# emmanuel-marty/zultra

Hardware: AMD Instinct MI355X
Metric: input MB/s, gzip 64 KiB max-blocks, enwik8-sized text, bit-exact vs CPU zultra (higher is better)
Workload: dtype u8/int32

## Files before the change

include/zultra_hip.h:

```cpp
#ifndef ZULTRA_HIP_H
#define ZULTRA_HIP_H

#include <stddef.h>
#include <stdint.h>

#ifdef __cplusplus
extern "C" {
#endif

typedef struct zultra_hip_ctx_s zultra_hip_ctx_t;

typedef struct zultra_hip_block_s {
   uint64_t win_off;
   uint32_t prev;
   uint32_t n;
} zultra_hip_block_t;

typedef struct zultra_hip_subblock_s {
   uint32_t block;
   uint32_t start;
   uint32_t size;
   uint32_t is_dynamic;
   int32_t static_cost;
   int32_t dynamic_cost;
// ... 19 lines not shown

double zultra_hip_copy_bandwidth(size_t nbytes, int iters);

zultra_hip_ctx_t *zultra_hip_create(int device, uint32_t max_block_size, uint32_t max_blocks);
void zultra_hip_destroy(zultra_hip_ctx_t *ctx);
const char *zultra_hip_last_error(const zultra_hip_ctx_t *ctx);

void zultra_hip_ctx_info(const zultra_hip_ctx_t *ctx, int *device, uint32_t *max_block_size, uint32_t *max_blocks, size_t *device_bytes);
size_t zultra_hip_context_bytes_on(int device, uint32_t max_block_size, uint32_t max_blocks);
size_t zultra_hip_context_bytes(uint32_t max_block_size, uint32_t max_blocks);

void *zultra_hip_staging(zultra_hip_ctx_t *ctx, int which, size_t size);

size_t zultra_hip_data_capacity(const zultra_hip_ctx_t *ctx);

int zultra_hip_compress_blocks(zultra_hip_ctx_t *ctx, const void *data, size_t data_size, int data_on_device,
                               const zultra_hip_block_t *blocks, uint32_t nblocks);

const zultra_hip_subblock_t *zultra_hip_subblocks(const zultra_hip_ctx_t *ctx, uint32_t *count);
const uint8_t *zultra_hip_payload(const zultra_hip_ctx_t *ctx, size_t *size);
void zultra_hip_last_timing(const zultra_hip_ctx_t *ctx, zultra_hip_timing_t *t);

typedef struct zultra_hip_stats_s {
   uint64_t positions, huge_positions;
   uint32_t blocks, subblocks, tasks, huge_tasks;
   uint32_t cut_tasks, cut_segments;
   uint32_t cut_redone;
   uint32_t runs;
   uint32_t settled_passes;
   uint32_t settled_kib;
   uint32_t cut_demoted;
   uint32_t runs_without_chain_kernels;
   uint32_t batches_rerun;
} zultra_hip_stats_t;
void zultra_hip_last_stats(const zultra_hip_ctx_t *ctx, zultra_hip_stats_t *out);

uint32_t zultra_hip_mf_chunk(const zultra_hip_ctx_t *ctx, uint32_t window_size, uint32_t *max_notes);

int zultra_hip_chain_trace(zultra_hip_ctx_t *ctx, uint64_t *out, uint32_t *slots);

int zultra_hip_cut_tasks(zultra_hip_ctx_t *ctx, uint32_t run, uint32_t *out, uint32_t cap);

int zultra_hip_get_matches(zultra_hip_ctx_t *ctx, uint32_t block, uint16_t *out);
int zultra_hip_get_splits(zultra_hip_ctx_t *ctx, uint32_t block, int *out );
int zultra_hip_get_parse(zultra_hip_ctx_t *ctx, uint32_t block, uint16_t *out);

typedef struct zultra_hip_bitstate_s {
   uint32_t acc;
   uint32_t nacc;
} zultra_hip_bitstate_t;

size_t zultra_hip_stitch(zultra_hip_bitstate_t *state, const zultra_hip_subblock_t *subs, uint32_t nsubs,
                         const uint8_t *payload, const uint8_t *raw, const uint64_t *raw_off, uint32_t max_block_size,
                         int final_block, uint8_t *out, size_t out_cap);
size_t zultra_hip_stitch_finish(zultra_hip_bitstate_t *state, uint8_t *out, size_t out_cap);

int zultra_hip_stitch_device(zultra_hip_ctx_t *ctx, zultra_hip_bitstate_t *state, int final_block, uint64_t *end_bit);
int zultra_hip_stitch_with_batch(zultra_hip_ctx_t *ctx, int enable, uint32_t phase, int final_block);
int zultra_hip_stitch_phase_table(zultra_hip_ctx_t *ctx, uint64_t *end_bits , uint32_t *failed_mask);
const void *zultra_hip_stream_device(const zultra_hip_ctx_t *ctx);
int zultra_hip_stream_read(zultra_hip_ctx_t *ctx, void *out, size_t offset, size_t nbytes);
int zultra_hip_stream_write(zultra_hip_ctx_t *ctx, const void *in, size_t offset, size_t nbytes);

#define ZULTRA_HIP_VERIFY_OK 0
typedef struct zultra_hip_verify_s {
   uint32_t bad_subblocks;
   uint32_t first_bad;
   uint32_t reason;
// ... 77 lines not shown
```

zultra_amd/_ffi.py:

```python
import ctypes as C

import numpy as np

ZULTRA_OK = 0
ZULTRA_STREAM_END = 1
ZULTRA_ERROR_SRC = -1
ZULTRA_ERROR_DST = -2
ZULTRA_ERROR_DICTIONARY = -3
ZULTRA_ERROR_MEMORY = -4
ZULTRA_ERROR_COMPRESSION = -5

FLAG_DEFLATE = 0
FLAG_ZLIB = 1
FLAG_GZIP = 2

CONTINUE = 0
FINALIZE = 1

_u8p = C.POINTER(C.c_uint8)
_SIZE_MAX = C.c_size_t(-1).value


class ZultraError(RuntimeError):
    pass


class _Stream(C.Structure):
    _fields_ = [("next_in", C.c_void_p), ("avail_in", C.c_size_t), ("total_in", C.c_ulonglong),
                ("next_out", C.c_void_p), ("avail_out", C.c_size_t), ("total_out", C.c_ulonglong),
                ("zalloc", C.c_void_p), ("zfree", C.c_void_p), ("opaque", C.c_void_p),
                ("state", C.c_void_p), ("adler", C.c_uint)]


class Block(C.Structure):
    _fields_ = [("win_off", C.c_uint64), ("prev", C.c_uint32), ("n", C.c_uint32)]


class SubBlock(C.Structure):
    _fields_ = [("block", C.c_uint32), ("start", C.c_uint32), ("size", C.c_uint32), ("is_dynamic", C.c_uint32),
                ("static_cost", C.c_int32), ("dynamic_cost", C.c_int32), ("failed", C.c_uint32), ("reserved", C.c_uint32),
                ("nbits", C.c_uint64), ("bits_off", C.c_uint64)]


class Timing(C.Structure):
    _fields_ = [(k, C.c_float) for k in ("h2d_ms", "matchfinder_ms", "tokenize_split_ms", "encode_ms", "d2h_ms", "total_ms",
                                         "group_ms", "frontier_ms", "stitch_ms", "init_ms", "parse_ms", "build_ms", "post_ms", "emit_ms", "head_ms", "tail_ms")]


class Stats(C.Structure):
    _fields_ = [("positions", C.c_uint64), ("huge_positions", C.c_uint64), ("blocks", C.c_uint32), ("subblocks", C.c_uint32),
                ("tasks", C.c_uint32), ("huge_tasks", C.c_uint32), ("cut_tasks", C.c_uint32), ("cut_segments", C.c_uint32),
                ("cut_redone", C.c_uint32), ("runs", C.c_uint32), ("settled_passes", C.c_uint32), ("settled_kib", C.c_uint32), ("cut_demoted", C.c_uint32),
                ("runs_without_chain_kernels", C.c_uint32), ("batches_rerun", C.c_uint32)]


class BitState(C.Structure):
    _fields_ = [("acc", C.c_uint32), ("nacc", C.c_uint32)]


class Verify(C.Structure):
    _fields_ = [("bad_subblocks", C.c_uint32), ("first_bad", C.c_uint32), ("reason", C.c_uint32), ("block", C.c_uint32),
                ("input_off", C.c_uint64), ("stream_bit", C.c_uint64), ("verified_bytes", C.c_uint64)]


class InflateItem(C.Structure):
    _fields_ = [("src_off", C.c_uint64), ("src_size", C.c_uint64), ("dst_off", C.c_uint64), ("dst_cap", C.c_uint64)]


class InflateResult(C.Structure):
    _fields_ = [("reason", C.c_uint32), ("blocks", C.c_uint32), ("out_size", C.c_uint64), ("src_used", C.c_uint64)]


class MemberResult(C.Structure):
    _fields_ = [("reason", C.c_uint32), ("blocks", C.c_uint32), ("out_size", C.c_uint64), ("src_used", C.c_uint64), ("head_size", C.c_uint32), ("check", C.c_uint32)]


class IndexResult(C.Structure):
    _fields_ = [("members", C.c_uint32), ("stop", C.c_uint32), ("out_size", C.c_uint64), ("src_used", C.c_uint64), ("tiles", C.c_uint32), ("tiles_rewalked", C.c_uint32)]


MEMBER_DTYPE = [("off", "<u8"), ("size", "<u8"), ("check", "<u4"), ("flags", "<u4")]
FRAME_BGZF = 4
ZIP_ENTRY_DTYPE = [("local_off", "<u8"), ("comp_size", "<u4"), ("size", "<u4"), ("crc32", "<u4"), ("name_len", "<u4")]
ZIP_EMPTY = 0xFFFFFFFF
MEMBER_RESULT_DTYPE = [("reason", "<u4"), ("blocks", "<u4"), ("out_size", "<u8"), ("src_used", "<u8"), ("head_size", "<u4"), ("check", "<u4")]


EXPORTS = [
    "zultra_stream_init", "zultra_stream_set_dictionary", "zultra_stream_compress", "zultra_stream_end",
    "zultra_memory_bound", "zultra_memory_compress", "zultra_memory_compress_dict", "zultra_set_device", "zultra_set_devices",
    "zultra_frame_get_header_size", "zultra_frame_encode_header", "zultra_frame_init_checksum",
    "zultra_frame_update_checksum", "zultra_frame_get_footer_size", "zultra_frame_encode_footer",
    "zultra_dictionary_load", "zultra_dictionary_free",
    "zultra_hip_device_count", "zultra_hip_selftest", "zultra_hip_traffic_probe", "zultra_hip_create", "zultra_hip_destroy", "zultra_hip_last_error",
    "zultra_hip_data_capacity", "zultra_hip_compress_blocks", "zultra_hip_subblocks", "zultra_hip_payload",
    "zultra_hip_last_timing", "zultra_hip_get_matches", "zultra_hip_get_splits", "zultra_hip_get_parse",
    "zultra_hip_stitch", "zultra_hip_stitch_finish",
    "zultra_hip_stitch_device", "zultra_hip_stitch_phase_table", "zultra_hip_stream_device", "zultra_hip_stream_read", "zultra_hip_block_crc32", "zultra_crc32_append", "zultra_crc32_append_many",
    "zultra_hip_create_files", "zultra_hip_compress_files", "zultra_hip_stitch_files", "zultra_hip_staging",
    "zultra_hip_block_adler32", "zultra_adler32_append", "zultra_hip_copy_bandwidth", "zultra_hip_last_stats", "zultra_hip_mf_chunk",
    "zultra_hip_ctx_info", "zultra_hip_context_bytes", "zultra_hip_context_bytes_on", "zultra_release_cached_contexts", "zultra_hip_chain_trace", "zultra_hip_cut_tasks", "zultra_hip_stitch_with_batch",
    "zultra_set_verify", "zultra_verified_bytes", "zultra_hip_verify_device", "zultra_hip_last_verify_ms", "zultra_hip_stream_write",
    "zultra_memory_decompress", "zultra_hip_inflate_streams", "zultra_memory_decompress_dict", "zultra_hip_inflate_streams_dict",
    "zultra_memory_decompress_batch", "zultra_hip_inflate_members",
    "zultra_hip_index_members", "zultra_hip_inflate_file", "zultra_memory_decompress_members",
    "zultra_hip_frame_members", "zultra_hip_last_frame_ms", "zultra_memory_bound_bgzf", "zultra_memory_compress_bgzf", "zultra_memory_compress_batch",
    "zultra_hip_zip_members", "zultra_hip_zip_device", "zultra_hip_zip_read", "zultra_hip_last_zip_ms",
    "zultra_zip_end_records", "zultra_memory_bound_zip", "zultra_memory_compress_zip",
]


def _as_u8(data):
    if isinstance(data, np.ndarray):
        return np.ascontiguousarray(data, dtype=np.uint8)
    return np.frombuffer(bytes(data), dtype=np.uint8)


class Lib:
    def __init__(self, path, allow_missing=()):
        self.path = path
        L = self.L = C.CDLL(path)
        missing = [n for n in EXPORTS if not hasattr(L, n) and n not in allow_missing]
        if missing:
            raise ZultraError("%s does not export %s" % (path, missing))
        L.zultra_stream_init.argtypes = [C.POINTER(_Stream), C.c_uint, C.c_uint]
        L.zultra_stream_init.restype = C.c_int
        L.zultra_stream_set_dictionary.argtypes = [C.POINTER(_Stream), C.c_void_p, C.c_int]
        L.zultra_stream_set_dictionary.restype = C.c_int
        L.zultra_stream_compress.argtypes = [C.POINTER(_Stream), C.c_int]
        L.zultra_stream_compress.restype = C.c_int
        L.zultra_stream_end.argtypes = [C.POINTER(_Stream)]
        L.zultra_stream_end.restype = None
        L.zultra_memory_bound.argtypes = [C.c_size_t, C.c_uint, C.c_uint]
# ... 12 lines not shown
        L.zultra_frame_get_header_size.argtypes = [C.c_uint, C.c_void_p, C.c_int]
        L.zultra_frame_get_footer_size.argtypes = [C.c_uint]
        L.zultra_hip_device_count.restype = C.c_int
        L.zultra_hip_create.argtypes = [C.c_int, C.c_uint32, C.c_uint32]
        L.zultra_hip_create.restype = C.c_void_p
        L.zultra_hip_destroy.argtypes = [C.c_void_p]
        L.zultra_hip_last_error.argtypes = [C.c_void_p]
        L.zultra_hip_last_error.restype = C.c_char_p
        L.zultra_hip_data_capacity.argtypes = [C.c_void_p]
        L.zultra_hip_data_capacity.restype = C.c_size_t
        L.zultra_hip_compress_blocks.argtypes = [C.c_void_p, C.c_void_p, C.c_size_t, C.c_int, C.POINTER(Block), C.c_uint32]
        L.zultra_hip_compress_blocks.restype = C.c_int
        L.zultra_hip_subblocks.argtypes = [C.c_void_p, C.POINTER(C.c_uint32)]
        L.zultra_hip_subblocks.restype = C.POINTER(SubBlock)
        L.zultra_hip_payload.argtypes = [C.c_void_p, C.POINTER(C.c_size_t)]
        L.zultra_hip_payload.restype = _u8p
        L.zultra_hip_last_timing.argtypes = [C.c_void_p, C.POINTER(Timing)]
        L.zultra_hip_get_matches.argtypes = [C.c_void_p, C.c_uint32, C.c_void_p]
        L.zultra_hip_get_splits.argtypes = [C.c_void_p, C.c_uint32, C.POINTER(C.c_int)]
        L.zultra_hip_get_parse.argtypes = [C.c_void_p, C.c_uint32, C.c_void_p]
        L.zultra_hip_stitch.argtypes = [C.POINTER(BitState), C.POINTER(SubBlock), C.c_uint32, C.c_void_p, C.c_void_p,
                                        C.POINTER(C.c_uint64), C.c_uint32, C.c_int, C.c_void_p, C.c_size_t]
        L.zultra_hip_stitch.restype = C.c_size_t
        L.zultra_hip_stitch_finish.argtypes = [C.POINTER(BitState), C.c_void_p, C.c_size_t]
        L.zultra_hip_stitch_finish.restype = C.c_size_t

    def device_count(self):
        return self.L.zultra_hip_device_count()

    def traffic_probe(self, nbytes):
        self.L.zultra_hip_traffic_probe.argtypes = [C.c_size_t]
        return self.L.zultra_hip_traffic_probe(nbytes)

    def copy_bandwidth(self, nbytes=1 << 30, iters=5):
        self.L.zultra_hip_copy_bandwidth.argtypes = [C.c_size_t, C.c_int]
        self.L.zultra_hip_copy_bandwidth.restype = C.c_double
        return self.L.zultra_hip_copy_bandwidth(nbytes, iters)

    def memory_bound(self, n, flags, max_block=0):
        return self.L.zultra_memory_bound(n, flags, max_block)

    def memory_compress(self, data, flags, max_block=0, dictionary=None, cap=None):
        data = _as_u8(data)
        if cap is None:
            cap = self.memory_bound(len(data), flags, max_block) + 16
        out = np.empty(max(cap, 1), dtype=np.uint8)
        if dictionary is not None and len(dictionary):
            d = _as_u8(dictionary)
            r = self.L.zultra_memory_compress_dict(data.ctypes.data, len(data), out.ctypes.data, cap, flags, max_block, d.ctypes.data, len(d))
        else:
            r = self.L.zultra_memory_compress(data.ctypes.data, len(data), out.ctypes.data, cap, flags, max_block)
        if r == _SIZE_MAX:
            return None
        return out[:r].tobytes()

    def memory_compress_into(self, data, flags, max_block, out):
        data = _as_u8(data)
        r = self.L.zultra_memory_compress(data.ctypes.data, len(data), out.ctypes.data, len(out), flags, max_block)
        return None if r == _SIZE_MAX else int(r)

    def memory_decompress(self, data, flags, max_out):
        data = _as_u8(data)
        out = np.empty(max(max_out, 1), dtype=np.uint8)
        f = self.L.zultra_memory_decompress
        f.argtypes = [C.c_void_p, C.c_size_t, C.c_void_p, C.c_size_t, C.c_uint]
        f.restype = C.c_size_t
# ... 549 lines not shown
```

zultra_amd/csrc/zh_device.hip:

```cpp
#include <zh_platform.h>

#include <stdio.h>
#include <stdlib.h>
#include <string.h>

#include <algorithm>
#include <mutex>
#include <vector>

#include "../../include/zultra_hip.h"
#include "zh_common.h"
#include "zh_host.h"
#include "zh_encode.h"
#include "zh_huffman.h"
#include "zh_matchfinder.h"
#include "zh_parse.h"
#include "zh_parse_chain.h"
#include "zh_parse_lanes.h"
#include "zh_split.h"
#include "zh_stitch.h"
#include "zh_frame.h"
#include "zh_zip.h"
#include "zh_verify.h"

// ... 97 lines not shown
   zh_bets_t bets;
   uint32_t streams_respread;
   uint32_t grid_cap;
   uint32_t mf_lds_cap;
   uint32_t *d_pay;
   uint32_t *d_tok_pos;
   uint16_t *d_tok_info;
   uint32_t *d_ntok, *d_split_tok, *d_split_cnt, *d_sub_base;
   uint32_t *d_chunkmax, *d_spanstart, *d_spancnt;
   uint32_t chunks_per_block;
   uint32_t *d_best;
   uint16_t *d_cost;
   zh_work_t *d_work;
   zh_subblock_t *d_results;
   uint8_t *d_payload;
   uint64_t *d_bars;
   uint64_t bar_stride, max_tasks;
   zh_sbstate_t *d_states;
   uint2 *d_taskmap;
   uint2 *d_taskinfo;
   uint32_t *d_ntasks, *d_hist_part, *d_task_bits;
   uint32_t *h_ntasks;
   uint32_t *d_hugelist;
   uint32_t *d_lanelist, *d_lane_acc;
   int lane_bundles;
   uint32_t lane_order, lane_tasks;
   uint4 *d_segtasks;
   uint2 *d_segitems;
   uint2 *d_segwaves;
   uint32_t demote_min;
   uint32_t coop_small;
   uint32_t seg_whole;
   int auto_runs;
   int last_runs;
   uint32_t seg_wide;
   int16_t *d_vecs;
   uint64_t seg_tasks_per_block, seg_items_per_block;
   uint64_t *d_chain_trace;
   int files_mode;
   uint32_t max_file_size;
   uint32_t max_subs;
   zh_graph_set_t batch_graph, run_graphs[2];
   uint64_t graph_tick;
   int files_run_graphs;
   int nlanes;
   hipStream_t lane_stream[ZH_MAX_RUNS];
   hipEvent_t lane_ev[ZH_MAX_RUNS][ZH_RUN_EVENTS];
   hipStream_t side_stream[ZH_MAX_RUNS];
   hipEvent_t side_ev[ZH_MAX_RUNS][8];
   hipEvent_t ev_input;
   hipEvent_t ev_fork;
   zh_subblock_t *d_results_compact;
   uint8_t *h_stage[2];
   size_t h_stage_size[2];
   uint32_t *h_crc;
   zh_block_t *h_blocks;
   zh_seg_t *h_segs;
   zh_subblock_t *h_results;
   zh_stitch_item_t *d_items;
   uint32_t *d_nsubs, *h_nsubs, *d_blk_start;
   zh_scan_out_t *d_scan_out, *h_scan_out;
   uint64_t *d_file_off;
   uint64_t *h_file_off;
   uint32_t *d_task_prefix, *h_task_prefix;
   uint32_t *d_stream;
   size_t stream_cap;
// ... 400 lines not shown
         return -1;
      }
   }
   if (kind == DEV) c->device_bytes += bytes;
   return 0;
}

static int zh_buffers(zultra_hip_ctx_t *c, zh_buf_op op, uint32_t sets) {
   const uint64_t B = c->max_blocks, S = c->segs_per_block, U = B * c->max_subs, T = c->max_tasks;
#define X(sets_, kind_, field_, count_) \
   if ((sets & (sets_)) && zh_buffer(c, op, kind_, #field_, (void **)&c->field_, (size_t)(count_) * sizeof(*c->field_))) return -1;
   ZH_CTX_BUFFERS(X)
#undef X
   return 0;
}
static uint32_t zh_creation_sets(int files_mode) {
   return ZH_SET_CORE | (files_mode ? ZH_SET_FILES : ZH_SET_BLOCKS) | (zh_env("ZULTRA_HIP_CHAIN_TRACE", 0) ? ZH_SET_TRACE : 0);
}

static int zh_need_file_off(zultra_hip_ctx_t *c) { return zh_buffers(c, ZH_BUF_ALLOC, ZH_SET_FILE_OFF); }
static int zh_need_events(zultra_hip_ctx_t *c, hipEvent_t *ev, int n) {
   for (int i = 0; i < n; i++)
      if (!ev[i]) ZH_CHECK(c, hipEventCreate(&ev[i]));
   return 0;
}
static int zh_need_verify(zultra_hip_ctx_t *c) { return zh_buffers(c, ZH_BUF_ALLOC, ZH_SET_VERIFY) || zh_need_events(c, c->ev_verify, 2); }
static int zh_need_frame(zultra_hip_ctx_t *c) { return zh_buffers(c, ZH_BUF_ALLOC, ZH_SET_FRAME) || zh_need_events(c, c->ev_frame, 4); }
static int zh_need_zip(zultra_hip_ctx_t *c) { return zh_buffers(c, ZH_BUF_ALLOC, ZH_SET_ZIP) || zh_need_events(c, c->ev_zip, 4); }
static void zh_drop_events(hipEvent_t *ev, int n) {
   for (int i = 0; i < n; i++)
      if (ev[i]) (void)hipEventDestroy(ev[i]);
}

extern "C" void zultra_hip_destroy(zultra_hip_ctx_t *c) {
   if (!c) return;
   (void)hipSetDevice(c->device);
   (void)zh_buffers(c, ZH_BUF_FREE, ZH_SET_ALL);
   for (int k = 0; k < ZH_MAX_RUNS; k++) {
      zh_drop_events(c->lane_ev[k], ZH_RUN_EVENTS);
      if (c->lane_stream[k]) (void)hipStreamDestroy(c->lane_stream[k]);
      zh_drop_events(c->side_ev[k], 8);
      if (c->side_stream[k]) (void)hipStreamDestroy(c->side_stream[k]);
   }
   zh_drop_events(&c->ev_input, 1);
   zh_drop_events(&c->ev_fork, 1);
   zh_graph_clear(&c->batch_graph);
   for (int i = 0; i < 2; i++) zh_graph_clear(&c->run_graphs[i]);
   zh_drop_events(c->ev_verify, 2);
   zh_drop_events(c->ev_frame, 4);
   zh_drop_events(c->ev_zip, 4);
   zh_drop_events(c->ev_stitch, ZH_STITCH_EVENTS);
   if (c->stream) (void)hipStreamDestroy(c->stream);
   delete c;
}

#ifndef ZH_EMU
__global__ void zh_queue_probe(uint64_t *out, uint64_t ticks) {
   const uint64_t t0 = zh_wall_clock();
   uint64_t t = t0;
   for (uint32_t guard = 0; t - t0 < ticks && guard < (1u << 20); guard++) {
      __builtin_amdgcn_s_sleep(64);
      t = zh_wall_clock();
   }
   out[0] = t0;
   out[1] = t;
}

static std::mutex g_probe_mutex;

static int zh_spread_streams(zultra_hip_ctx_t *c) {
   if (zh_env("ZULTRA_HIP_SPREAD_STREAMS", 0) <= 0) return 0;
   std::lock_guard<std::mutex> probe_lock(g_probe_mutex);
   const int n = c->nlanes;
   hipStream_t *order[2 * ZH_MAX_RUNS];
   bool high[2 * ZH_MAX_RUNS];
   int m = 0;
   const int scope = zh_env("ZULTRA_HIP_SPREAD_SCOPE", 0);
   for (int k = 0; k < n && k < 3; k++) { order[m] = &c->lane_stream[k]; high[m++] = false; }
   if (scope >= 1) for (int k = 0; k < n && k < 3; k++) { order[m] = &c->side_stream[k]; high[m++] = true; }
   for (int k = 3; k < n; k++) { order[m] = &c->lane_stream[k]; high[m++] = false; }
   if (scope >= 1) for (int k = 3; k < n; k++) { order[m] = &c->side_stream[k]; high[m++] = true; }
   uint64_t *d_t = NULL, *h_t = NULL;
   ZH_CHECK(c, hipMalloc((void **)&d_t, (size_t)m * 2 * sizeof(uint64_t)));
   ZH_CHECK(c, hipHostMalloc((void **)&h_t, (size_t)m * 2 * sizeof(uint64_t), 0));
   int lo_prio = 0, hi_prio = 0;
   (void)hipDeviceGetStreamPriorityRange(&lo_prio, &hi_prio);
   int rc = 0;
   c->streams_respread = 0;
   for (int attempt = 0; attempt < 12; attempt++) {
      for (int i = 0; i < m; i++) hipLaunchKernelGGL(zh_queue_probe, dim3(1), dim3(1), 0, *order[i], d_t + 2 * i, (uint64_t)20000);
      for (int i = 0; i < m; i++) if (hipStreamSynchronize(*order[i]) != hipSuccess) rc = -1;
      if (rc != 0 || hipMemcpy(h_t, d_t, (size_t)m * 2 * sizeof(uint64_t), hipMemcpyDeviceToHost) != hipSuccess) { rc = -1; break; }
      int bad = -1;
      for (int i = 1; i < m && bad < 0; i++)
         for (int j = 0; j < i; j++)
            if (!(h_t[2 * i] < h_t[2 * j + 1] && h_t[2 * j] < h_t[2 * i + 1])) {
               const uint64_t gap_ij = h_t[2 * i] >= h_t[2 * j + 1] ? h_t[2 * i] - h_t[2 * j + 1] : ~0ull, gap_ji = h_t[2 * j] >= h_t[2 * i + 1] ? h_t[2 * j] - h_t[2 * i + 1] : ~0ull;
               if (gap_ij <= 3000u || gap_ji <= 3000u) { bad = i; break; }
            }
      if (bad < 0) break;
      hipStream_t fresh = NULL;
      const hipError_t e = high[bad] ? hipStreamCreateWithPriority(&fresh, hipStreamNonBlocking, hi_prio) : hipStreamCreateWithFlags(&fresh, hipStreamNonBlocking);
      if (e != hipSuccess) { rc = -1; break; }
      (void)hipStreamDestroy(*order[bad]);
      *order[bad] = fresh;
      c->streams_respread++;
   }
   (void)hipFree(d_t);
   (void)hipHostFree(h_t);
   if (zh_env("ZULTRA_HIP_SPREAD_STREAMS", 0) == 2) fprintf(stderr, "zultra_amd: %u of %d streams replaced for a hardware queue of their own\n", c->streams_respread, m);
   if (rc != 0) snprintf(c->err, sizeof(c->err), "stream placement probe failed");
   return rc;
}
#endif

static zh_stitch_job_t zh_job_stream(uint32_t phase, int final_block, bool scan_only = false) { return {phase & 7u, final_block, false, scan_only, false, {0, 0}}; }
static zh_stitch_job_t zh_job_files(void) { return {0, -1, true, false, false, {0, 0}}; }
static zh_stitch_job_t zh_job_framed(uint32_t framing, uint32_t eof) { return {0, -1, true, false, true, {framing, eof}}; }
static int zh_enqueue_stitch(zultra_hip_ctx_t *c, hipStream_t st, const zh_stitch_job_t &job, bool clear);
static int zh_stitch_verdict(zultra_hip_ctx_t *c, bool scan_only);

static void zh_assembly_clear(zultra_hip_ctx_t *c) { c->held = zh_assembly_t{}; }
static void zh_assembly_record(zultra_hip_ctx_t *c, const zh_stitch_job_t &job, bool with_batch, int rc) {
   zh_assembly_clear(c);
   if (job.scan_only || (rc != 0 && !with_batch)) return;
   const uint32_t gap = job.framed ? zh_frame_head(job.frame.framing) + zh_frame_tail(job.frame.framing) : 0u;
   c->held = {job.files ? ZH_LAYOUT_FILES : ZH_LAYOUT_STREAM, job.phase, job.final_block, gap, with_batch, rc};
}
static bool zh_assembly_usable(const zultra_hip_ctx_t *c) { return c->held.layout != ZH_LAYOUT_NONE && c->held.rc == 0; }
static bool zh_assembly_is_files(const zultra_hip_ctx_t *c) { return c->held.layout == ZH_LAYOUT_FILES; }
static uint32_t zh_assembly_gap(const zultra_hip_ctx_t *c) { return c->held.gap; }
static bool zh_assembly_plain_files(const zultra_hip_ctx_t *c) { return zh_assembly_usable(c) && zh_assembly_is_files(c) && zh_assembly_gap(c) == 0; }
static bool zh_assembly_brought(const zultra_hip_ctx_t *c, const zh_stitch_job_t &job, int *rc) {
   const zh_assembly_t &h = c->held;
   if (!h.with_batch || h.layout != (job.files ? ZH_LAYOUT_FILES : ZH_LAYOUT_STREAM) || (!job.files && (h.phase != job.phase || h.final_block != job.final_block))) return false;
   *rc = h.rc;
   return true;
}

static int zh_env_lanes(void) {
   const int streams = zh_env("ZULTRA_HIP_STREAMS", 0);
   return streams > 0 ? min(streams, (int)ZH_MAX_RUNS) : 4;
}

static uint32_t zh_env_mf_cap(void) { return (uint32_t)max((int)ZH_MFL_MINCAP, zh_env("ZULTRA_HIP_MF_CAP", (int)ZH_MFL_CAP_LIMIT)); }

static int zh_create_buffers(zultra_hip_ctx_t *c) {
   ZH_CHECK(c, hipSetDevice(c->device));
   {
      static std::mutex checked_mutex;
      static uint64_t checked_ok[4] = {0, 0, 0, 0};
      std::lock_guard<std::mutex> lock(checked_mutex);
      const uint32_t dv = (uint32_t)c->device & 255u;
      if (!((checked_ok[dv >> 6] >> (dv & 63u)) & 1ull)) {
         const int bad = zultra_hip_selftest();
         if (bad != 0) {
            snprintf(c->err, sizeof(c->err), "device %d fails the self-check of the wave and LDS primitives (%d)", c->device, bad);
            return -1;
         }
         checked_ok[dv >> 6] |= 1ull << (dv & 63u);
      }
   }
   ZH_CHECK(c, hipFuncSetAttribute(reinterpret_cast<const void *>(&zh_mf_group<true>), hipFuncAttributeMaxDynamicSharedMemorySize, ZH_MF_GROUP_LDS));
   ZH_CHECK(c, hipFuncSetAttribute(reinterpret_cast<const void *>(&zh_mf_frontier<true>), hipFuncAttributeMaxDynamicSharedMemorySize, ZH_MF_FRONTIER_LDS));
   ZH_CHECK(c, hipFuncSetAttribute(reinterpret_cast<const void *>(&zh_mf_group_big), hipFuncAttributeMaxDynamicSharedMemorySize, ZH_MF_GROUP_LDS));
   ZH_CHECK(c, hipStreamCreate(&c->stream));
   for (int i = 0; i < ZH_STITCH_EVENTS; i++) ZH_CHECK(c, hipEventCreate(&c->ev_stitch[i]));
   ZH_CHECK(c, hipEventCreate(&c->ev_fork));
   {
      c->demote_min = (uint32_t)zh_env("ZULTRA_HIP_DEMOTE", 2);
      c->coop_small = (uint32_t)zh_env("ZULTRA_HIP_COOP_SMALL", 256);
      if (c->coop_small < 64u) c->coop_small = 64u;
      if (c->coop_small > ZH_COOP_MIN) c->coop_small = ZH_COOP_MIN;
      c->seg_whole = (uint32_t)zh_env("ZULTRA_HIP_SEG_WHOLE", 16384);
      c->bets.on = zh_env("ZULTRA_HIP_CHAIN_SKIP", 1);
      c->bets.seen_runs = 0;
      c->grid_cap = (uint32_t)max(0, zh_env("ZULTRA_HIP_GRID_CAP", 0));
      c->lane_order = zh_env("ZULTRA_HIP_LANE_ORDER", 1) != 0;
      c->lane_bundles = zh_env("ZULTRA_HIP_LANE_BUNDLES", 1) != 0;
      c->lane_tasks = (uint32_t)min(max(0, zh_env("ZULTRA_HIP_LANE_TASKS", 0)), (int)ZH_LP_TASKS);
      c->seg_wide = (uint32_t)zh_env("ZULTRA_HIP_SEG_WIDE", 1024);
      if (zh_mfl_note_room(c->sort_stride, c->run_stride) < c->seg_W / zh_mfl_cap(c->seg_W, c->mf_lds_cap)) {
         snprintf(c->err, sizeof(c->err), "matchfinder note table too small for chunks of %u", c->mf_lds_cap);
         return -1;
      }
      const int streams = zh_env("ZULTRA_HIP_STREAMS", 0);
      c->auto_runs = streams > 0 ? 0 : 1;
      c->files_run_graphs = zh_env("ZULTRA_HIP_FILES_RUN_GRAPHS", 1);
      for (int k = 0; k < c->nlanes; k++) {
         ZH_CHECK(c, hipStreamCreateWithFlags(&c->lane_stream[k], hipStreamNonBlocking));
         for (int i = 0; i < ZH_RUN_EVENTS; i++) ZH_CHECK(c, hipEventCreate(&c->lane_ev[k][i]));
         {
            int lo_prio = 0, hi_prio = 0;
            (void)hipDeviceGetStreamPriorityRange(&lo_prio, &hi_prio);
            ZH_CHECK(c, hipStreamCreateWithPriority(&c->side_stream[k], hipStreamNonBlocking, hi_prio));
         }
         for (int i = 0; i < 8; i++) ZH_CHECK(c, hipEventCreate(&c->side_ev[k][i]));
      }
      ZH_CHECK(c, hipEventCreate(&c->ev_input));
#ifndef ZH_EMU
      if (zh_spread_streams(c) != 0) return -1;
#endif
   }
   if (zh_buffers(c, ZH_BUF_ALLOC, zh_creation_sets(c->files_mode))) return -1;
   if (c->d_chain_trace) ZH_CHECK(c, hipMemset(c->d_chain_trace, 0, ZH_TRACE_WORDS * sizeof(uint64_t)));
   memset(c->h_nsubs, 0, (1 + ZH_MAX_RUNS) * sizeof(uint32_t));
   memset(c->h_ntasks, 0, 2 * ZH_NCNT * sizeof(uint32_t));
   ZH_CHECK(c, hipMemset(c->d_ntasks, 0, ZH_NCNT * sizeof(uint32_t)));
   {
      std::vector<uint32_t> t(256 + 1024);
      for (uint32_t i = 0; i < 256; i++) {
         uint32_t v = i;
         for (int k = 0; k < 8; k++) v = (v >> 1) ^ ((v & 1) ? 0xEDB88320u : 0);
         t[i] = v;
      }
      for (int b = 0; b < 4; b++)
         for (uint32_t i = 0; i < 256; i++) {
            uint32_t v = i << (8 * b);
            for (int k = 0; k < ZH_CRC_SLICE; k++) v = (v >> 8) ^ t[v & 0xff];
            t[256 + 256 * b + i] = v;
         }
      ZH_CHECK(c, hipMemcpy(c->d_crc_tables, t.data(), t.size() * sizeof(uint32_t), hipMemcpyHostToDevice));
   }
   return 0;
}

static zultra_hip_ctx_t *zh_create(int device, uint32_t max_block, uint32_t max_blocks, int files_mode) {
   int ndev = zultra_hip_device_count();
   if (ndev <= 0 || device < 0 || device >= ndev || max_blocks == 0) return NULL;
   zultra_hip_ctx_t *c = new zultra_hip_ctx_s();
   memset((void *)&c->timing, 0, sizeof(c->timing));
   c->device = device;
   zh_shape(c, max_block, max_blocks, files_mode, zh_device_cus(device), zh_env_lanes(), zh_env_mf_cap());
   c->err[0] = 0;
   if (zh_create_buffers(c) != 0) {
// ... 446 lines not shown
   memcpy(c->crc.data(), c->h_crc, nblocks * sizeof(uint32_t));
   c->adler.assign(c->h_adler, c->h_adler + 2 * (size_t)nblocks);
   c->nsubs = nblocks;
   zh_assembly_record(c, zh_job_files(), true, zh_stitch_verdict(c, false));
   (void)hipEventElapsedTime(&c->timing.h2d_ms, c->lane_ev[0][ZH_EV_START], c->ev_input);
   (void)hipEventElapsedTime(&c->timing.encode_ms, c->lane_ev[0][ZH_EV_INPUT], c->lane_ev[0][ZH_EV_READBACK]);
   (void)hipEventElapsedTime(&c->timing.total_ms, c->lane_ev[0][ZH_EV_START], c->lane_ev[0][ZH_EV_READBACK]);
   return (int)nblocks;
}


static int zh_check_batch(zultra_hip_ctx_t *c, const void *data, size_t data_size, int data_on_device, const zultra_hip_block_t *blocks, uint32_t nblocks) {
   if (!c || !data || !blocks || nblocks == 0 || nblocks > c->max_blocks) {
      if (c) snprintf(c->err, sizeof(c->err), "bad arguments");
      return -1;
   }
   for (uint32_t b = 0; b < nblocks; b++) {
      if (blocks[b].n == 0 || blocks[b].n > c->max_block || (c->files_mode && (blocks[b].n > c->max_file_size || blocks[b].prev != 0)) || blocks[b].prev > ZH_HISTORY || (uint64_t)blocks[b].prev + blocks[b].n > c->W ||
          blocks[b].win_off + blocks[b].prev + blocks[b].n > data_size) {
         snprintf(c->err, sizeof(c->err), "block %u out of range", b);
         return -1;
      }
   }
   if (data_on_device != 1 && data_size > c->data_cap) {
      snprintf(c->err, sizeof(c->err), "batch of %zu bytes exceeds the context's staging capacity %zu", data_size, c->data_cap);
      return -1;
   }
   return 0;
}

static void zh_plan_runs(zultra_hip_ctx_t *c, const zultra_hip_block_t *blocks, uint32_t nblocks, uint32_t *run_b0 ) {
   uint64_t batch_bytes = 0;
   for (uint32_t b = 0; b < nblocks; b++) batch_bytes += blocks[b].n;
   const uint64_t want_runs = c->auto_runs ? (batch_bytes >= (256ull << 20) ? 4u : 3u) : (uint64_t)c->nlanes;
   const int lanes = c->last_runs = (int)zh_max64(1, zh_min64(want_runs, zh_min64((uint64_t)nblocks / 4u, batch_bytes >> 22)));
   const uint32_t share = nblocks / (uint32_t)lanes;
   run_b0[0] = 0;
   for (int k = 1; k < lanes; k++)
      run_b0[k] = k == 1 ? share : k == lanes - 1 ? nblocks - share : share + (uint32_t)((uint64_t)(nblocks - 2u * share) * (uint64_t)(k - 1) / (uint64_t)(lanes - 2));
   run_b0[lanes] = nblocks;
}

static int zh_upload_batch(zultra_hip_ctx_t *c, const void *data, size_t data_size, int data_on_device, const zultra_hip_block_t *blocks, uint32_t nblocks, uint8_t **stage) {
   hipStream_t st0 = c->lane_stream[0];
   ZH_CHECK(c, hipEventRecord(c->lane_ev[0][ZH_EV_START], st0));
   *stage = NULL;
   if (data_on_device == 2 && !c->files_mode) {
      *stage = (uint8_t *)zultra_hip_staging(c, 0, data_size);
      if (!*stage) {
         snprintf(c->err, sizeof(c->err), "no pinned staging for %zu bytes", data_size);
         return -1;
      }
   }
   if (data_on_device == 1)
      c->cur_data = (const uint8_t *)data;
   else {
      if (!*stage) ZH_CHECK(c, hipMemcpyAsync(c->d_data, data, data_size, hipMemcpyHostToDevice, st0));
      c->cur_data = c->d_data;
   }
   memcpy(c->h_blocks, blocks, nblocks * sizeof(zh_block_t));
   ZH_CHECK(c, hipMemcpyAsync(c->d_blocks, c->h_blocks, nblocks * sizeof(zh_block_t), hipMemcpyHostToDevice, st0));
   if (c->files_mode) {
      uint32_t acc = 0;
      for (uint32_t b = 0; b < nblocks; b++) {
         c->h_task_prefix[b] = acc;
         acc += (blocks[b].n + ZH_TASK - 1) / ZH_TASK;
      }
      c->h_task_prefix[nblocks] = acc;
// ... 559 lines not shown
   if (!c || (int)run >= c->last_runs || c->files_mode) return -1;
   const uint32_t n = min(cap, c->h_ntasks[(size_t)run * ZH_CNT_STRIDE + ZH_CNT_SEGTASKS]);
   if (out && n) ZH_CHECK(c, hipMemcpy(out, c->d_segtasks + (uint64_t)c->bets.run[run].b0 * c->seg_tasks_per_block, (size_t)n * sizeof(uint4), hipMemcpyDeviceToHost));
   return (int)n;
}

extern "C" uint32_t zultra_hip_mf_chunk(const zultra_hip_ctx_t *c, uint32_t window_size, uint32_t *max_notes) {
   if (!c) return 0;
   if (max_notes) *max_notes = zh_mfl_note_room(c->sort_stride, c->run_stride);
   return zh_mfl_cap(min(window_size, (uint32_t)ZH_SEG_WINDOW), c->mf_lds_cap);
}

extern "C" void zultra_hip_last_stats(const zultra_hip_ctx_t *c, zultra_hip_stats_t *out) {
   if (!c || !out) return;
   memset(out, 0, sizeof(*out));
   out->blocks = c->nblocks;
   out->subblocks = c->nsubs;
   out->batches_rerun = c->bets.reruns;
   for (int k = 0; k < c->last_runs && k < ZH_MAX_RUNS; k++) {
      const uint32_t *cnt = c->h_ntasks + (size_t)k * ZH_CNT_STRIDE;
      out->tasks += cnt[ZH_CNT_TASKS];
      out->huge_tasks += cnt[ZH_CNT_VLONG] + cnt[ZH_CNT_LONG] + cnt[ZH_CNT_SHORT] + cnt[ZH_CNT_SEGTASKS];
      out->huge_positions += cnt[ZH_CNT_HUGE_POS];
      out->cut_tasks += cnt[ZH_CNT_SEGTASKS];
      out->cut_segments += cnt[ZH_CNT_SEGITEMS];
      out->cut_redone += cnt[ZH_CNT_SEG_FAILED];
      out->cut_demoted += cnt[ZH_CNT_DEMOTED];
      out->runs_without_chain_kernels += cnt[ZH_CNT_NOCHAINS] ? 1u : 0u;
      out->settled_passes += cnt[ZH_CNT_SETTLED];
      out->settled_kib += cnt[ZH_CNT_SETTLED_POS];
   }
   for (uint32_t b = 0; b < c->nblocks; b++) out->positions += c->blocks[b].n;
   out->runs = (uint32_t)c->last_runs;
}

extern "C" int zultra_hip_get_matches(zultra_hip_ctx_t *c, uint32_t block, uint16_t *out) {
   if (!c || block >= c->nblocks) return -1;
   ZH_CHECK(c, hipSetDevice(c->device));
   const size_t n = c->blocks[block].n;
   std::vector<uint32_t> lo(n * 4), hi(n * 4);
   const uint32_t *base = (const uint32_t *)(c->d_match + (uint64_t)block * c->match_stride);
   ZH_CHECK(c, hipMemcpy(lo.data(), base, n * 16, hipMemcpyDeviceToHost));
   ZH_CHECK(c, hipMemcpy(hi.data(), base + 4 * ZH_ROW_HI_OFF(c->match_stride), n * 16, hipMemcpyDeviceToHost));
   uint32_t *o = (uint32_t *)out;
   for (size_t i = 0; i < n; i++) {
      const bool more = (lo[4 * i + 3] & 0xffffu) >= ZH_MIN_MATCH;
      for (int k = 0; k < 4; k++) {
         o[8 * i + k] = lo[4 * i + k];
         o[8 * i + 4 + k] = more ? hi[4 * i + k] : 0u;
      }
   }
   return 0;
}

extern "C" int zultra_hip_get_splits(zultra_hip_ctx_t *c, uint32_t block, int *out) {
   if (!c || block >= c->nblocks) return -1;
   ZH_CHECK(c, hipSetDevice(c->device));
   uint32_t st[ZH_MAX_SPLITS + 1], nt = 0, cnt = 0;
   ZH_CHECK(c, hipMemcpy(&cnt, c->d_split_cnt + block, sizeof(cnt), hipMemcpyDeviceToHost));
   if (cnt > ZH_MAX_SPLITS) return -1;
   ZH_CHECK(c, hipMemcpy(st, c->d_split_tok + (uint64_t)block * (ZH_MAX_SPLITS + 1), sizeof(st), hipMemcpyDeviceToHost));
   ZH_CHECK(c, hipMemcpy(&nt, c->d_ntok + block, sizeof(nt), hipMemcpyDeviceToHost));
   for (uint32_t k = 0; k < cnt; k++) {
      uint32_t t1 = st[k + 1], pos = c->blocks[block].prev + c->blocks[block].n;
      if (t1 < nt) ZH_CHECK(c, hipMemcpy(&pos, c->d_tok_pos + (uint64_t)block * c->tok_stride + t1, sizeof(pos), hipMemcpyDeviceToHost));
      out[k] = (int)pos;
// ... 16 lines not shown
```

Baseline: 2225.

## Create run streams lazily and probe hardware queue collisions at context creation

Run streams are now created only up to the number of runs the context can use. A new probe launches timing kernels on the lane and side streams to find pairs that share a hardware queue. For three runs it swaps streams so the lone colliding run sits in the middle slot, and it records a fitted run count. The default stream is created after the run streams, so queue assignment order changes. This aims to stop concurrent runs from serialising on a shared hardware queue, at the cost of a startup probe. runs_fitted is computed but zh_plan_runs does not read it yet.

```diff
diff --git a/include/zultra_hip.h b/include/zultra_hip.h
--- a/include/zultra_hip.h
+++ b/include/zultra_hip.h
@@ -75,8 +75,12 @@
    uint32_t cut_demoted;
    uint32_t runs_without_chain_kernels;
    uint32_t batches_rerun;
+   uint32_t runs_fitted;
+   uint32_t stream_collisions;
 } zultra_hip_stats_t;
 void zultra_hip_last_stats(const zultra_hip_ctx_t *ctx, zultra_hip_stats_t *out);
+
+uint32_t zultra_hip_runs_for(uint64_t batch_bytes, uint32_t nblocks, int streams_setting);
 
 uint32_t zultra_hip_mf_chunk(const zultra_hip_ctx_t *ctx, uint32_t window_size, uint32_t *max_notes);
 
diff --git a/zultra_amd/_ffi.py b/zultra_amd/_ffi.py
--- a/zultra_amd/_ffi.py
+++ b/zultra_amd/_ffi.py
@@ -51,7 +51,7 @@
     _fields_ = [("positions", C.c_uint64), ("huge_positions", C.c_uint64), ("blocks", C.c_uint32), ("subblocks", C.c_uint32),
                 ("tasks", C.c_uint32), ("huge_tasks", C.c_uint32), ("cut_tasks", C.c_uint32), ("cut_segments", C.c_uint32),
                 ("cut_redone", C.c_uint32), ("runs", C.c_uint32), ("settled_passes", C.c_uint32), ("settled_kib", C.c_uint32), ("cut_demoted", C.c_uint32),
-                ("runs_without_chain_kernels", C.c_uint32), ("batches_rerun", C.c_uint32)]
+                ("runs_without_chain_kernels", C.c_uint32), ("batches_rerun", C.c_uint32), ("runs_fitted", C.c_uint32), ("stream_collisions", C.c_uint32)]
 
 
 class BitState(C.Structure):
@@ -98,7 +98,7 @@
     "zultra_hip_stitch", "zultra_hip_stitch_finish",
     "zultra_hip_stitch_device", "zultra_hip_stitch_phase_table", "zultra_hip_stream_device", "zultra_hip_stream_read", "zultra_hip_block_crc32", "zultra_crc32_append", "zultra_crc32_append_many",
     "zultra_hip_create_files", "zultra_hip_compress_files", "zultra_hip_stitch_files", "zultra_hip_staging",
-    "zultra_hip_block_adler32", "zultra_adler32_append", "zultra_hip_copy_bandwidth", "zultra_hip_last_stats", "zultra_hip_mf_chunk",
+    "zultra_hip_block_adler32", "zultra_adler32_append", "zultra_hip_copy_bandwidth", "zultra_hip_last_stats", "zultra_hip_runs_for", "zultra_hip_mf_chunk",
     "zultra_hip_ctx_info", "zultra_hip_context_bytes", "zultra_hip_context_bytes_on", "zultra_release_cached_contexts", "zultra_hip_chain_trace", "zultra_hip_cut_tasks", "zultra_hip_stitch_with_batch",
     "zultra_set_verify", "zultra_verified_bytes", "zultra_hip_verify_device", "zultra_hip_last_verify_ms", "zultra_hip_stream_write",
     "zultra_memory_decompress", "zultra_hip_inflate_streams", "zultra_memory_decompress_dict", "zultra_hip_inflate_streams_dict",
@@ -177,6 +177,11 @@
         self.L.zultra_hip_traffic_probe.argtypes = [C.c_size_t]
         return self.L.zultra_hip_traffic_probe(nbytes)
 
+    def runs_for(self, batch_bytes, nblocks, streams_setting=0):
+        self.L.zultra_hip_runs_for.argtypes = [C.c_uint64, C.c_uint32, C.c_int]
+        self.L.zultra_hip_runs_for.restype = C.c_uint32
+        return int(self.L.zultra_hip_runs_for(batch_bytes, nblocks, streams_setting))
+
     def copy_bandwidth(self, nbytes=1 << 30, iters=5):
         self.L.zultra_hip_copy_bandwidth.argtypes = [C.c_size_t, C.c_int]
         self.L.zultra_hip_copy_bandwidth.restype = C.c_double
diff --git a/zultra_amd/csrc/zh_device.hip b/zultra_amd/csrc/zh_device.hip
--- a/zultra_amd/csrc/zh_device.hip
+++ b/zultra_amd/csrc/zh_device.hip
@@ -153,6 +153,10 @@
    uint32_t coop_small;
    uint32_t seg_whole;
    int auto_runs;
+   int streams_setting;
+   int run_pairs;
+   int runs_fitted;
+   uint32_t stream_collisions;
    int last_runs;
    uint32_t seg_wide;
    int16_t *d_vecs;
@@ -619,16 +623,34 @@
       if (ev[i]) (void)hipEventDestroy(ev[i]);
 }
 
+static int zh_need_run_streams(zultra_hip_ctx_t *c, int runs) {
+   for (int k = c->run_pairs; k < runs && k < ZH_MAX_RUNS; k++, c->run_pairs++) {
+      ZH_CHECK(c, hipStreamCreateWithFlags(&c->lane_stream[k], hipStreamNonBlocking));
+      if (zh_need_events(c, c->lane_ev[k], ZH_RUN_EVENTS)) return -1;
+      {
+         int lo_prio = 0, hi_prio = 0;
+         (void)hipDeviceGetStreamPriorityRange(&lo_prio, &hi_prio);
+         ZH_CHECK(c, hipStreamCreateWithPriority(&c->side_stream[k], hipStreamNonBlocking, hi_prio));
+      }
+      if (zh_need_events(c, c->side_ev[k], 8)) return -1;
+   }
+   return 0;
+}
+static void zh_drop_run_streams(zultra_hip_ctx_t *c, int k) {
+   zh_drop_events(c->lane_ev[k], ZH_RUN_EVENTS);
+   zh_drop_events(c->side_ev[k], 8);
+   if (c->lane_stream[k]) (void)hipStreamDestroy(c->lane_stream[k]);
+   if (c->side_stream[k]) (void)hipStreamDestroy(c->side_stream[k]);
+   for (int i = 0; i < ZH_RUN_EVENTS; i++) c->lane_ev[k][i] = NULL;
+   for (int i = 0; i < 8; i++) c->side_ev[k][i] = NULL;
+   c->lane_stream[k] = c->side_stream[k] = NULL;
+}
+
 extern "C" void zultra_hip_destroy(zultra_hip_ctx_t *c) {
    if (!c) return;
    (void)hipSetDevice(c->device);
    (void)zh_buffers(c, ZH_BUF_FREE, ZH_SET_ALL);
-   for (int k = 0; k < ZH_MAX_RUNS; k++) {
-      zh_drop_events(c->lane_ev[k], ZH_RUN_EVENTS);
-      if (c->lane_stream[k]) (void)hipStreamDestroy(c->lane_stream[k]);
-      zh_drop_events(c->side_ev[k], 8);
-      if (c->side_stream[k]) (void)hipStreamDestroy(c->side_stream[k]);
-   }
+   for (int k = 0; k < ZH_MAX_RUNS; k++) zh_drop_run_streams(c, k);
    zh_drop_events(&c->ev_input, 1);
    zh_drop_events(&c->ev_fork, 1);
    zh_graph_clear(&c->batch_graph);
@@ -655,10 +677,31 @@
 
 static std::mutex g_probe_mutex;
 
+static int zh_probe_streams(hipStream_t *const *order, int m, uint64_t *d_t, uint64_t *h_t, int *first_bad, uint64_t *shared = NULL) {
+   for (int i = 0; i < m; i++) hipLaunchKernelGGL(zh_queue_probe, dim3(1), dim3(1), 0, *order[i], d_t + 2 * i, (uint64_t)20000);
+   bool failed = false;
+   for (int i = 0; i < m; i++) failed |= hipStreamSynchronize(*order[i]) != hipSuccess;
+   if (failed || hipMemcpy(h_t, d_t, (size_t)m * 2 * sizeof(uint64_t), hipMemcpyDeviceToHost) != hipSuccess) return -1;
+   int pairs = 0;
+   *first_bad = -1;
+   if (shared) *shared = 0;
+   for (int i = 1; i < m; i++)
+      for (int j = 0; j < i; j++)
+         if (!(h_t[2 * i] < h_t[2 * j + 1] && h_t[2 * j] < h_t[2 * i + 1])) {
+            const uint64_t gap_ij = h_t[2 * i] >= h_t[2 * j + 1] ? h_t[2 * i] - h_t[2 * j + 1] : ~0ull, gap_ji = h_t[2 * j] >= h_t[2 * i + 1] ? h_t[2 * j] - h_t[2 * i + 1] : ~0ull;
+            if (gap_ij <= 3000u || gap_ji <= 3000u) {
+               if (*first_bad < 0) *first_bad = i;
+               if (shared && i < 4) *shared |= 1ull << (i * 16 + j);
+               pairs++;
+            }
+         }
+   return pairs;
+}
+
 static int zh_spread_streams(zultra_hip_ctx_t *c) {
    if (zh_env("ZULTRA_HIP_SPREAD_STREAMS", 0) <= 0) return 0;
    std::lock_guard<std::mutex> probe_lock(g_probe_mutex);
-   const int n = c->nlanes;
+   const int n = c->run_pairs;
    hipStream_t *order[2 * ZH_MAX_RUNS];
    bool high[2 * ZH_MAX_RUNS];
    int m = 0;
@@ -675,16 +718,8 @@
    int rc = 0;
    c->streams_respread = 0;
    for (int attempt = 0; attempt < 12; attempt++) {
-      for (int i = 0; i < m; i++) hipLaunchKernelGGL(zh_queue_probe, dim3(1), dim3(1), 0, *order[i], d_t + 2 * i, (uint64_t)20000);
-      for (int i = 0; i < m; i++) if (hipStreamSynchronize(*order[i]) != hipSuccess) rc = -1;
-      if (rc != 0 || hipMemcpy(h_t, d_t, (size_t)m * 2 * sizeof(uint64_t), hipMemcpyDeviceToHost) != hipSuccess) { rc = -1; break; }
       int bad = -1;
-      for (int i = 1; i < m && bad < 0; i++)
-         for (int j = 0; j < i; j++)
-            if (!(h_t[2 * i] < h_t[2 * j + 1] && h_t[2 * j] < h_t[2 * i + 1])) {
-               const uint64_t gap_ij = h_t[2 * i] >= h_t[2 * j + 1] ? h_t[2 * i] - h_t[2 * j + 1] : ~0ull, gap_ji = h_t[2 * j] >= h_t[2 * i + 1] ? h_t[2 * j] - h_t[2 * i + 1] : ~0ull;
-               if (gap_ij <= 3000u || gap_ji <= 3000u) { bad = i; break; }
-            }
+      if (zh_probe_streams(order, m, d_t, h_t, &bad) < 0) { rc = -1; break; }
       if (bad < 0) break;
       hipStream_t fresh = NULL;
       const hipError_t e = high[bad] ? hipStreamCreateWithPriority(&fresh, hipStreamNonBlocking, hi_prio) : hipStreamCreateWithFlags(&fresh, hipStreamNonBlocking);
@@ -698,6 +733,40 @@
    if (zh_env("ZULTRA_HIP_SPREAD_STREAMS", 0) == 2) fprintf(stderr, "zultra_amd: %u of %d streams replaced for a hardware queue of their own\n", c->streams_respread, m);
    if (rc != 0) snprintf(c->err, sizeof(c->err), "stream placement probe failed");
    return rc;
+}
+
+static int zh_look_at_streams(zultra_hip_ctx_t *c) {
+   if (c->files_mode || !c->auto_runs || c->runs_fitted < 2) return 0;
+   std::lock_guard<std::mutex> probe_lock(g_probe_mutex);
+   uint64_t *d_t = NULL, *h_t = NULL;
+   ZH_CHECK(c, hipMalloc((void **)&d_t, (size_t)4 * c->runs_fitted * sizeof(uint64_t)));
+   if (hipHostMalloc((void **)&h_t, (size_t)4 * c->runs_fitted * sizeof(uint64_t), 0) != hipSuccess) {
+      (void)hipFree(d_t);
+      snprintf(c->err, sizeof(c->err), "stream placement probe: no pinned memory");
+      return -1;
+   }
+   int pairs = 0;
+   for (int R = c->runs_fitted, first = 1; R >= 1; R--, first = 0) {
+      hipStream_t *order[2 * ZH_MAX_RUNS];
+      for (int k = 0; k < R; k++) order[k] = &c->lane_stream[k], order[R + k] = &c->side_stream[k];
+      int first_bad = -1;
+      uint64_t shared = 0;
+      pairs = zh_probe_streams(order, 2 * R, d_t, h_t, &first_bad, &shared);
+      if (pairs < 0) break;
+      if (first) c->stream_collisions = (uint32_t)pairs;
+      if (first && R == 3) {
+         const bool s10 = (shared >> 16) & 1u, s20 = (shared >> 32) & 1u, s21 = (shared >> 33) & 1u;
+         const int lone = (s21 && !s10 && !s20) ? 0 : (s10 && !s20 && !s21) ? 2 : 1;
+         std::swap(c->lane_stream[1], c->lane_stream[lone]);
+         std::swap(c->side_stream[1], c->side_stream[lone]);
+      }
+      c->runs_fitted = R;
+      if (pairs == 0) break;
+   }
+   (void)hipFree(d_t);
+   (void)hipHostFree(h_t);
+   if (pairs < 0) snprintf(c->err, sizeof(c->err), "stream placement probe failed");
+   return pairs < 0 ? -1 : 0;
 }
 #endif
 
@@ -728,6 +797,11 @@
 static int zh_env_lanes(void) {
    const int streams = zh_env("ZULTRA_HIP_STREAMS", 0);
    return streams > 0 ? min(streams, (int)ZH_MAX_RUNS) : 4;
+}
+
+extern "C" uint32_t zultra_hip_runs_for(uint64_t batch_bytes, uint32_t nblocks, int streams_setting) {
+   uint64_t want = streams_setting > 0 ? (uint64_t)min(streams_setting, (int)ZH_MAX_RUNS) : batch_bytes >= (256ull << 20) ? 4u : 3u;
+   return (uint32_t)zh_max64(1, zh_min64(want, zh_min64((uint64_t)nblocks / 4u, batch_bytes >> 22)));
 }
 
 static uint32_t zh_env_mf_cap(void) { return (uint32_t)max((int)ZH_MFL_MINCAP, zh_env("ZULTRA_HIP_MF_CAP", (int)ZH_MFL_CAP_LIMIT)); }
@@ -751,7 +825,6 @@
    ZH_CHECK(c, hipFuncSetAttribute(reinterpret_cast<const void *>(&zh_mf_group<true>), hipFuncAttributeMaxDynamicSharedMemorySize, ZH_MF_GROUP_LDS));
    ZH_CHECK(c, hipFuncSetAttribute(reinterpret_cast<const void *>(&zh_mf_frontier<true>), hipFuncAttributeMaxDynamicSharedMemorySize, ZH_MF_FRONTIER_LDS));
    ZH_CHECK(c, hipFuncSetAttribute(reinterpret_cast<const void *>(&zh_mf_group_big), hipFuncAttributeMaxDynamicSharedMemorySize, ZH_MF_GROUP_LDS));
-   ZH_CHECK(c, hipStreamCreate(&c->stream));
    for (int i = 0; i < ZH_STITCH_EVENTS; i++) ZH_CHECK(c, hipEventCreate(&c->ev_stitch[i]));
    ZH_CHECK(c, hipEventCreate(&c->ev_fork));
    {
@@ -772,22 +845,18 @@
          return -1;
       }
       const int streams = zh_env("ZULTRA_HIP_STREAMS", 0);
+      c->streams_setting = max(streams, 0);
       c->auto_runs = streams > 0 ? 0 : 1;
       c->files_run_graphs = zh_env("ZULTRA_HIP_FILES_RUN_GRAPHS", 1);
-      for (int k = 0; k < c->nlanes; k++) {
-         ZH_CHECK(c, hipStreamCreateWithFlags(&c->lane_stream[k], hipStreamNonBlocking));
-         for (int i = 0; i < ZH_RUN_EVENTS; i++) ZH_CHECK(c, hipEventCreate(&c->lane_ev[k][i]));
-         {
-            int lo_prio = 0, hi_prio = 0;
-            (void)hipDeviceGetStreamPriorityRange(&lo_prio, &hi_prio);
-            ZH_CHECK(c, hipStreamCreateWithPriority(&c->side_stream[k], hipStreamNonBlocking, hi_prio));
-         }
-         for (int i = 0; i < 8; i++) ZH_CHECK(c, hipEventCreate(&c->side_ev[k][i]));
-      }
+      if (c->files_mode) ZH_CHECK(c, hipStreamCreate(&c->stream));
+      const int most = (int)zultra_hip_runs_for((uint64_t)c->max_blocks * c->max_block, c->max_blocks, c->streams_setting);
+      if (zh_need_run_streams(c, c->files_mode || (c->auto_runs && most > 1) ? c->nlanes : most) != 0) return -1;
+      c->runs_fitted = min(min(c->run_pairs, most), 3);
       ZH_CHECK(c, hipEventCreate(&c->ev_input));
 #ifndef ZH_EMU
-      if (zh_spread_streams(c) != 0) return -1;
+      if (zh_spread_streams(c) != 0 || zh_look_at_streams(c) != 0) return -1;
 #endif
+      if (!c->stream) ZH_CHECK(c, hipStreamCreate(&c->stream));
    }
    if (zh_buffers(c, ZH_BUF_ALLOC, zh_creation_sets(c->files_mode))) return -1;
    if (c->d_chain_trace) ZH_CHECK(c, hipMemset(c->d_chain_trace, 0, ZH_TRACE_WORDS * sizeof(uint64_t)));
@@ -1300,8 +1369,7 @@
 static void zh_plan_runs(zultra_hip_ctx_t *c, const zultra_hip_block_t *blocks, uint32_t nblocks, uint32_t *run_b0 ) {
    uint64_t batch_bytes = 0;
    for (uint32_t b = 0; b < nblocks; b++) batch_bytes += blocks[b].n;
-   const uint64_t want_runs = c->auto_runs ? (batch_bytes >= (256ull << 20) ? 4u : 3u) : (uint64_t)c->nlanes;
-   const int lanes = c->last_runs = (int)zh_max64(1, zh_min64(want_runs, zh_min64((uint64_t)nblocks / 4u, batch_bytes >> 22)));
+   const int lanes = c->last_runs = (int)zultra_hip_runs_for(batch_bytes, nblocks, c->streams_setting);
    const uint32_t share = nblocks / (uint32_t)lanes;
    run_b0[0] = 0;
    for (int k = 1; k < lanes; k++)
@@ -1927,6 +1995,8 @@
    }
    for (uint32_t b = 0; b < c->nblocks; b++) out->positions += c->blocks[b].n;
    out->runs = (uint32_t)c->last_runs;
+   out->runs_fitted = (uint32_t)c->runs_fitted;
+   out->stream_collisions = c->stream_collisions;
 }
 
 extern "C" int zultra_hip_get_matches(zultra_hip_ctx_t *c, uint32_t block, uint16_t *out) {
```

New measurement: 2717 (median of 6 runs). 22.1% higher.
